# CESNET/GPUJPEG

Measured on AMD Instinct MI355X. Metric: Mpix/s encode+decode (8K RGB q75), higher is better.
Workload: dtype f32

## Files before the change

### gpujpeg_amd/csrc/gj_dec_idct.hip

```cpp
#include "gj_dec_internal.h"

__global__ __launch_bounds__(256) void k_idct(const gj_geom g, int16_t* __restrict__ coefs, const float* __restrict__ qtab,
                                              uint8_t* __restrict__ planes, const int zero)
{
    if (g.fb.sizes != nullptr) {
        coefs += (size_t)blockIdx.z * g.fb.coefs;
        planes += (size_t)blockIdx.z * g.fb.coefs;
    }
    const unsigned gb = blockIdx.x * 256u + threadIdx.x;
    if (gb >= (unsigned)g.block_count) return;
    unsigned bx, by;
    const gj_comp_geom& k = g.comp[gj_block_of(g, gb, bx, by)];
    uint32_t w[32];
    {
        uint4* p = reinterpret_cast<uint4*>(coefs + (size_t)gb * 64);
#pragma unroll
        for (int r = 0; r < 8; r++) {
            const uint4 v = p[r];
            if (zero) p[r] = make_uint4(0, 0, 0, 0);
            w[r * 4] = v.x; w[r * 4 + 1] = v.y; w[r * 4 + 2] = v.z; w[r * 4 + 3] = v.w;
        }
    }
    uint32_t px[16];
    gj_idct_pk(w, qtab + k.q_table * 64, px);
// ... 84 lines not shown
    const unsigned lb = lb0 + threadIdx.x;
    const unsigned nchunk = min(256u, nb - lb0) * 8u;
    const unsigned by = lb / (unsigned)k0.blocks_x, bx = lb - by * (unsigned)k0.blocks_x;
    uint32_t pk[3][16];
#pragma unroll
    for (int c = 0; c < 3; c++) {
        uint4* src = reinterpret_cast<uint4*>(coefs + g.comp[c].data_offset + (size_t)lb0 * 64);
        uint4 w[8];
#pragma unroll
        for (int i = 0; i < 8; i++) {
            const unsigned ch = i * 256u + threadIdx.x;
            w[i] = ch < nchunk ? src[ch] : make_uint4(0, 0, 0, 0);
        }
        if (zero) {
#pragma unroll
            for (int i = 0; i < 8; i++) {
                const unsigned ch = i * 256u + threadIdx.x;
                if (ch < nchunk) src[ch] = make_uint4(0, 0, 0, 0);
            }
        }
        if (c) __syncthreads();
#pragma unroll
        for (int i = 0; i < 8; i++) {
            const unsigned ch = i * 256u + threadIdx.x;
            *reinterpret_cast<uint4*>(s_blk + (ch >> 3) * GJ_TILE_PITCH + (ch & 7u) * 16u) = w[i];
        }
        __syncthreads();
        uint32_t wb[32];
        {
            const uint4* p = reinterpret_cast<const uint4*>(s_blk + threadIdx.x * GJ_TILE_PITCH);
#pragma unroll
            for (int r = 0; r < 8; r++) {
                const uint4 v = p[r];
                wb[r * 4] = v.x; wb[r * 4 + 1] = v.y; wb[r * 4 + 2] = v.z; wb[r * 4 + 3] = v.w;
            }
        }
        gj_idct_pk(wb, s_q[c], pk[c]);
#pragma unroll
        for (int i = 0; i < 16; i++) GJ_KEEP(pk[c][i]);
    }
    gj_store_rgb444<CS_FROM, CS_TO>(g, raw, pk, lb, nb, bx, by);
}

__device__ __forceinline__ uint4* gj_slot_row(uint8_t* slot, const int lane, const int r)
{
    return reinterpret_cast<uint4*>(slot + ((uint32_t)(r << 4) ^ (((uint32_t)lane & 7u) << 4)));
}

__device__ __forceinline__ void gj_slot_put(uint8_t* slot, const uint32_t swz , const uint32_t tok)
{
    reinterpret_cast<uint16_t*>(slot)[(tok & 63u) ^ swz] = (uint16_t)(tok & 0xFFC0u);
}

template <bool MULTI>
__device__ __forceinline__ void gj_tok_to_slot(uint8_t* slot, uint16_t* stage, const int lane, const bool fast, const uint32_t S, const uint32_t start,
                                               const uint32_t cnt, const uint32_t dc, const bool in_plane, const uint4* __restrict__ plane_block,
                                               const uint16_t* __restrict__ d_tok)
{
#pragma unroll
    for (int r = 0; r < 8; r++) *gj_slot_row(slot, lane, r) = make_uint4(0, 0, 0, 0);
    if (in_plane) {
#pragma unroll
        for (int r = 0; r < 8; r++) *gj_slot_row(slot, lane, r) = plane_block[r];
    }
    const uint32_t end = start + cnt;
    const uint32_t swz = ((uint32_t)lane & 7u) << 3;
    if (fast) {
        gj_wave_sync();
        uint32_t a = start - S;
        const uint32_t b = end - S;
        for (; a + 2 <= b; a += 2) {
            const uint32_t ta = stage[a], tb = stage[a + 1];
            gj_slot_put(slot, swz, ta);
            gj_slot_put(slot, swz, tb);
        }
        if (a < b) gj_slot_put(slot, swz, stage[a]);
    } else {
        const uint32_t prev_end = (uint32_t)__builtin_amdgcn_update_dpp(0, (int)end, 0x138, 0xF, 0xF, false);
        const unsigned long long runs0 = __ballot(lane == 0 || start != prev_end);
        uint32_t total = 0, my_at = 0;
        for (unsigned long long runs = MULTI ? runs0 : 0ull; runs;) {
            const int d = __builtin_ctzll(runs);
            runs &= runs - 1;
            const int dn = runs ? __builtin_ctzll(runs) : 64;
            const uint32_t RS = (uint32_t)__builtin_amdgcn_readlane((int)start, d), RE = (uint32_t)__builtin_amdgcn_readlane((int)end, dn - 1);
            if (lane >= d && lane < dn) my_at = total + (start - (RS & ~7u));
            total += RE > (RS & ~7u) ? (RE - (RS & ~7u) + 7u) & ~7u : 0u;
            if (RE < RS) total = GJ_TOK_STAGE + 1u;
        }
        if (MULTI && total <= GJ_TOK_STAGE) {
            gj_wave_sync();
            uint32_t at = 0;
            for (unsigned long long runs = runs0; runs;) {
                const int d = __builtin_ctzll(runs);
                runs &= runs - 1;
                const int dn = runs ? __builtin_ctzll(runs) : 64;
                const uint32_t RS = (uint32_t)__builtin_amdgcn_readlane((int)start, d) & ~7u, RE = (uint32_t)__builtin_amdgcn_readlane((int)end, dn - 1);
                for (uint32_t i = (uint32_t)lane * 8u; RS + i < RE; i += 512u)
                    *reinterpret_cast<uint4*>(stage + at + i) = *reinterpret_cast<const uint4*>(d_tok + RS + i);
                at += RE > RS ? (RE - RS + 7u) & ~7u : 0u;
            }
            gj_wave_sync();
            for (uint32_t a = 0; a < cnt; a++) gj_slot_put(slot, swz, stage[my_at + a]);
        } else {
            unsigned long long runs = runs0;
            while (runs) {
                const int d = __builtin_ctzll(runs);
                runs &= runs - 1;
                const int dn = runs ? __builtin_ctzll(runs) : 64;
                const uint32_t RS = (uint32_t)__builtin_amdgcn_readlane((int)start, d), RE = (uint32_t)__builtin_amdgcn_readlane((int)end, dn - 1);
                const bool mine = lane >= d && lane < dn;
                for (uint32_t base = RS & ~7u; base < RE; base += GJ_TOK_STAGE) {
                    gj_wave_sync();
                    for (uint32_t i = (uint32_t)lane * 8u; i < GJ_TOK_STAGE && base + i < RE; i += 512u)
                        *reinterpret_cast<uint4*>(stage + i) = *reinterpret_cast<const uint4*>(d_tok + base + i);
                    gj_wave_sync();
                    if (mine) {
                        const uint32_t b = min(end, base + GJ_TOK_STAGE);
                        for (uint32_t a = max(start, base); a < b; a++) gj_slot_put(slot, swz, stage[a - base]);
                    }
                }
            }
        }
    }
    if (!in_plane) *reinterpret_cast<uint16_t*>(slot + ((lane & 7) << 4)) = (uint16_t)dc;
    gj_wave_sync();
}

struct __attribute__((aligned(16))) GjTokLds {
    uint8_t blk[256 * 128];
    uint16_t stage[4][GJ_TOK_STAGE];
    float q[2][3][64];
};

__device__ __forceinline__ void gj_tok_tables(GjTokLds& s, const gj_geom& g, const float* __restrict__ qtab)
{
    if (threadIdx.x < 192) {
        const float q = qtab[g.comp[threadIdx.x >> 6].q_table * 64 + (threadIdx.x & 63)];
        s.q[0][threadIdx.x >> 6][threadIdx.x & 63] = (threadIdx.x & 63) ? q * 0.015625f : q;
        s.q[1][threadIdx.x >> 6][threadIdx.x & 63] = q;
    }
}

__device__ __forceinline__ void gj_tok_idct3(GjTokLds& s, const gj_geom& g, const int16_t* __restrict__ coefs, const uint16_t* __restrict__ d_tok,
                                             const unsigned lb, const uint32_t (&start)[3], const uint32_t (&cd)[3], uint32_t (&pk)[3][16])
{
    const int lane = threadIdx.x & 63;
    uint8_t* slot = s.blk + threadIdx.x * 128;
    uint16_t* stage = s.stage[threadIdx.x >> 6];
    GjTokRange cur = gj_tok_fetch(d_tok, start[0], gj_rec_count(cd[0]), lane);
#pragma unroll
    for (int c = 0; c < 3; c++) {
        const bool fast = cur.fast;
        const uint32_t S = cur.S;
        if (fast) {
            *reinterpret_cast<uint4*>(stage + lane * 8) = cur.t0;
            if (lane * 8 + 512 < GJ_TOK_STAGE) *reinterpret_cast<uint4*>(stage + lane * 8 + 512) = cur.t1;
        }
        if (c < 2) cur = gj_tok_fetch(d_tok, start[c + 1], gj_rec_count(cd[c + 1]), lane);
        const bool in_plane = (int32_t)cd[c] < 0;
        gj_tok_to_slot<false>(slot, stage, lane, fast, S, start[c], gj_rec_count(cd[c]), cd[c] & 0xFFFFu, in_plane,
                       reinterpret_cast<const uint4*>(coefs + g.comp[c].data_offset + (size_t)lb * 64), d_tok);
        uint32_t wb[32];
#pragma unroll
        for (int r = 0; r < 8; r++) {
            const uint4 v = *gj_slot_row(slot, lane, r);
            wb[r * 4] = v.x; wb[r * 4 + 1] = v.y; wb[r * 4 + 2] = v.z; wb[r * 4 + 3] = v.w;
        }
        gj_idct_pk(wb, s.q[in_plane ? 1 : 0][c], pk[c]);
#pragma unroll
        for (int i = 0; i < 16; i++) GJ_KEEP(pk[c][i]);
    }
}

template <int CS_FROM, int CS_TO>
__global__ __launch_bounds__(256, 4) void k_idct_tok_rgb444(const gj_geom g, const int16_t* __restrict__ coefs, const uint2* __restrict__ d_rec,
                                                            const uint16_t* __restrict__ d_tok, const uint32_t tok_cap,
                                                            const float* __restrict__ qtab, uint8_t* __restrict__ raw)
{
    if (g.fb.sizes != nullptr) {
        const size_t z = blockIdx.z;
        coefs += z * g.fb.coefs; d_rec += z * g.fb.rec; d_tok += z * g.fb.tok;
        raw += z * g.fb.raw;
    }
    __shared__ GjTokLds s;
    gj_tok_tables(s, g, qtab);
    const gj_comp_geom& k0 = g.comp[0];
    const unsigned nb = (unsigned)(k0.blocks_x * k0.blocks_y);
    const unsigned lb = blockIdx.x * 256u + threadIdx.x;
    const unsigned by = lb / (unsigned)k0.blocks_x, bx = lb - by * (unsigned)k0.blocks_x;
    uint32_t start[3], cd[3];
#pragma unroll
    for (int c = 0; c < 3; c++) gj_tok_record(g, d_rec, tok_cap, lb < nb, lb, c, start[c], cd[c]);
    __syncthreads();
    uint32_t pk[3][16];
    gj_tok_idct3(s, g, coefs, d_tok, lb, start, cd, pk);
    gj_store_rgb444<CS_FROM, CS_TO>(g, raw, pk, lb, nb, bx, by);
}

template <int CS_FROM, int CS_TO, bool BATCH>
__global__ __launch_bounds__(256, 4) void k_idct_tok_region_rgb444(const gj_geom g, const gj_geom gr, const gj_region rg_in, const int16_t* __restrict__ coefs,
                                                                   const uint2* __restrict__ d_rec, const uint16_t* __restrict__ d_tok,
                                                                   const uint32_t tok_cap, const float* __restrict__ qtab, uint8_t* __restrict__ raw)
{
    if (BATCH) {
        const size_t z = blockIdx.z;
        coefs += z * g.fb.coefs; d_rec += z * g.fb.rec; d_tok += z * g.fb.tok;
        raw += z * g.fb.raw;
    }
    const gj_region_frame& rg = BATCH ? rg_in.d_frames[blockIdx.z] : rg_in.frame;
    __shared__ GjTokLds s;
    gj_tok_tables(s, g, qtab);
    const int lane = threadIdx.x & 63;
    const unsigned cbx = (unsigned)(rg.bx1[0] - rg.bx0[0]), cby = (unsigned)(rg.by1[0] - rg.by0[0]);
    const unsigned pieces = (cbx + 63u) / 64u;
    const unsigned gw = blockIdx.x * 4u + (threadIdx.x >> 6);
    const unsigned crow = gw / pieces, piece = gw - crow * pieces;
    const unsigned in_piece = crow < cby ? min(64u, cbx - piece * 64u) : 0u;
    const bool valid = (unsigned)lane < in_piece;
    const unsigned fby = (unsigned)rg.by0[0] + min(crow, cby - 1u);
    const unsigned fbx = (unsigned)rg.bx0[0] + piece * 64u + (valid ? (unsigned)lane : (in_piece ? in_piece - 1u : 0u));
    const unsigned lb = fby * (unsigned)g.comp[0].blocks_x + fbx;
    uint32_t start[3], cd[3];
#pragma unroll
    for (int c = 0; c < 3; c++) gj_tok_record(g, d_rec, tok_cap, true, lb, c, start[c], cd[c]);
    if (!valid) {
#pragma unroll
        for (int c = 0; c < 3; c++) {
            start[c] += gj_rec_count(cd[c]);
            cd[c] = 0;
        }
    }
    __syncthreads();
    uint32_t pk[3][16];
    gj_tok_idct3(s, g, coefs, d_tok, lb, start, cd, pk);
    if (!valid) return;
    const int W = gr.width, H = gr.height;
    const size_t pitch = (size_t)W * 3 + gr.width_padding;
    const int x0 = (int)(fbx * 8u) - rg.x, y0 = (int)(fby * 8u) - rg.y;
    const bool inside = x0 >= 0 && x0 + 8 <= W;
#pragma unroll
    for (int r = 0; r < 8; r++) {
        uint32_t px[6] = {0, 0, 0, 0, 0, 0};
        const uint32_t c0[2] = {pk[0][2 * r], pk[0][2 * r + 1]}, c1[2] = {pk[1][2 * r], pk[1][2 * r + 1]}, c2[2] = {pk[2][2 * r], pk[2][2 * r + 1]};
        gj_store_pair<CS_FROM, CS_TO, 0>(c0, c1, c2, px);
        gj_store_pair<CS_FROM, CS_TO, 2>(c0, c1, c2, px);
        gj_store_pair<CS_FROM, CS_TO, 4>(c0, c1, c2, px);
        gj_store_pair<CS_FROM, CS_TO, 6>(c0, c1, c2, px);
        const int y = y0 + r;
        if (y >= 0 && y < H) {
            uint8_t* row = raw + (size_t)y * pitch;
            uint8_t* p = row + (ptrdiff_t)x0 * 3;
            if (inside && (reinterpret_cast<uintptr_t>(p) & 3) == 0) {
                uint32_t* q = reinterpret_cast<uint32_t*>(p);
#pragma unroll
                for (int i = 0; i < 6; i++) q[i] = px[i];
            } else {
#pragma unroll
                for (int byte = 0; byte < 24; byte++) {
                    const int x = x0 + byte / 3;
                    if (x >= 0 && x < W) row[(size_t)x * 3 + byte % 3] = (uint8_t)(px[byte >> 2] >> ((byte & 3) * 8));
                }
            }
        }
        __builtin_amdgcn_sched_barrier(0);
    }
}

__global__ __launch_bounds__(256, 4) void k_idct_tok_uyvy422(const gj_geom g, const int16_t* __restrict__ coefs, const uint2* __restrict__ d_rec,
                                                             const uint16_t* __restrict__ d_tok, const uint32_t tok_cap,
                                                             const float* __restrict__ qtab, uint8_t* __restrict__ raw)
{
    if (g.fb.sizes != nullptr) {
        const size_t z = blockIdx.z;
        coefs += z * g.fb.coefs; d_rec += z * g.fb.rec; d_tok += z * g.fb.tok;
        raw += z * g.fb.raw;
    }
    __shared__ GjTokLds s;
    gj_tok_tables(s, g, qtab);
    const gj_comp_geom& kc = g.comp[1];
    const unsigned nm = (unsigned)(kc.blocks_x * kc.blocks_y);
    const int p = threadIdx.x & 3;
    const unsigned m = blockIdx.x * 64u + (threadIdx.x >> 2);
    const unsigned my = m / (unsigned)kc.blocks_x, mx = m - my * (unsigned)kc.blocks_x;
    const int c = p < 2 ? 0 : p - 1;
    const int lane = threadIdx.x & 63;
    uint8_t* slot = s.blk + threadIdx.x * 128;
    uint16_t* stage = s.stage[threadIdx.x >> 6];
    uint32_t start = 0, cnt = 0, dc = 0;
    bool in_plane = false;
    if (m < nm) {
        const uint2 r = d_rec[(size_t)m * 4 + p];
        const uint32_t cd = gj_rec_pack(r, tok_cap);
        start = r.x;
        cnt = gj_rec_count(cd);
        dc = cd & 0xFFFFu;
        in_plane = (int32_t)cd < 0;
    }
    const GjTokRange tr = gj_tok_fetch(d_tok, start, cnt, lane);
    if (tr.fast) {
        *reinterpret_cast<uint4*>(stage + lane * 8) = tr.t0;
        if (lane * 8 + 512 < GJ_TOK_STAGE) *reinterpret_cast<uint4*>(stage + lane * 8 + 512) = tr.t1;
    }
    __syncthreads();
    const size_t blk = p < 2 ? (size_t)my * g.comp[0].blocks_x + 2 * mx + p : (size_t)m;
    gj_tok_to_slot<true>(slot, stage, lane, tr.fast, tr.S, start, cnt, dc, in_plane,
                   reinterpret_cast<const uint4*>(coefs + g.comp[c].data_offset + (m < nm ? blk : 0) * 64), d_tok);
    uint32_t wb[32];
#pragma unroll
    for (int r = 0; r < 8; r++) {
        const uint4 v = *gj_slot_row(slot, lane, r);
        wb[r * 4] = v.x; wb[r * 4 + 1] = v.y; wb[r * 4 + 2] = v.z; wb[r * 4 + 3] = v.w;
    }
    uint32_t px[16];
    gj_idct_pk(wb, s.q[in_plane ? 1 : 0][c], px);

    const size_t pitch = (size_t)g.width * 2 + g.width_padding;
    const bool interior = m < nm && (mx * 16 + 16 <= (unsigned)g.width) && (my * 8 + 8 <= (unsigned)g.height);
    const bool aligned = ((pitch | (size_t)raw) & 7) == 0;
    const uint32_t sel_uv = (p & 1) ? 0x07030602u : 0x05010400u;
#pragma unroll
    for (int r = 0; r < 8; r++) {
        const int a0 = (int)px[2 * r], a1 = (int)px[2 * r + 1];
        const uint32_t y00 = (uint32_t)__builtin_amdgcn_update_dpp(0, a0, 0x00, 0xF, 0xF, false), y01 = (uint32_t)__builtin_amdgcn_update_dpp(0, a1, 0x00, 0xF, 0xF, false);
// ... 167 lines not shown
bool gj_is_uyvy422(const gj_geom& g)
{
    return g.pixel_format == GJ_PF_422_P1020 && g.comp_count == 3 &&
           (g.color_space == g.color_space_internal || g.color_space == GJ_CS_NONE || g.color_space_internal == GJ_CS_NONE) &&
           g.comp[0].samp_h == 2 && g.comp[0].samp_v == 1 && g.comp[1].samp_h == 1 && g.comp[1].samp_v == 1 && g.comp[2].samp_h == 1 &&
           g.comp[2].samp_v == 1 && g.comp[0].blocks_x == 2 * g.comp[1].blocks_x && g.comp[0].blocks_y == g.comp[1].blocks_y &&
           g.comp[2].blocks_x == g.comp[1].blocks_x && g.comp[2].blocks_y == g.comp[1].blocks_y;
}

gj_idct_tok_t gj_idct_tok_for(const gj_geom& g)
{
    if (!g.interleaved) return gj_idct_tok_kernel(g);
    if (gj_is_uyvy422(g) && g.blocks_per_mcu == 4 && g.mcu_count == g.comp[1].blocks_x * g.comp[1].blocks_y && g.mcu_comp[0] == 0 && g.mcu_comp[1] == 0 &&
        g.mcu_comp[2] == 1 && g.mcu_comp[3] == 2 && g.mcu_bx[0] == 0 && g.mcu_bx[1] == 1)
        return k_idct_tok_uyvy422;
    return nullptr;
}

extern "C" int gj_hip_decode_uses_planes(const gj_geom* g, int use_fused)
{
    return !(use_fused && (gj_is_uyvy422(*g) || gj_idct_fused_kernel(*g) != nullptr));
}

static void gj_launch_postprocess(const gj_geom& g, const gj_dec_job* job, hipStream_t st, const unsigned frames)
{
    if (g.no_transform) {
        hipLaunchKernelGGL(k_copy_planes_out, dim3(2048, 1, frames), dim3(256), 0, st, g, job->d_planes, job->d_raw);
    } else {
        const unsigned n = (unsigned)g.raw_width * (unsigned)g.height;
        hipLaunchKernelGGL(k_postprocess, dim3((n + 255) / 256, 1, frames), dim3(256), 0, st, g, job->d_planes, job->d_raw);
    }
}

void gj_launch_idct(const gj_dec_job* job, hipStream_t st, gj_idct_tok_t idct_tok, gj_event_t* ev)
{
    const gj_geom& g = job->g;
    const bool tokens = idct_tok != nullptr;
    const unsigned frames = job->batch.count > 1 ? job->batch.count : 1u;
    int path = 0;
    const char* what = "idct / postprocess";
    if (job->region.on) {
        gj_launch_idct_region(job, st, tokens, ev);
        path = tokens ? 4 : 3;
        what = job->region.d_frames ? "idct / postprocess (batch of regions)" : "idct / postprocess (region)";
    } else if (job->scale > 1) {
        const bool done = gj_launch_idct_scaled(job, st, tokens);
        if (ev) GJ_HIP_CHECK(hipEventRecord((hipEvent_t)ev[2], st));
        if (!done) gj_launch_postprocess(job->gs, job, st, frames);
        path = done ? 2 : 1;
        what = "idct / postprocess (reduced size)";
    } else if (tokens) {
        const unsigned nb = g.interleaved ? (unsigned)g.block_count : (unsigned)(g.comp[0].blocks_x * g.comp[0].blocks_y);
        hipLaunchKernelGGL(idct_tok, dim3((nb + 255) / 256, 1, frames), dim3(256), 0, st, g, job->d_coefs, (const uint2*)job->d_blkrec, (const uint16_t*)job->d_tok, job->tok_cap,
                           job->d_qtabf, job->d_raw);
        if (ev) GJ_HIP_CHECK(hipEventRecord((hipEvent_t)ev[2], st));
    } else if (job->use_fused && gj_is_uyvy422(g)) {
        const unsigned nm = (unsigned)(g.comp[1].blocks_x * g.comp[1].blocks_y);
        hipLaunchKernelGGL(k_idct_fused_uyvy422, dim3((nm + 255) / 256, 1, frames), dim3(256), 0, st, g, job->d_coefs, job->d_qtabf, job->d_raw, job->zero_coefs);
        if (ev) GJ_HIP_CHECK(hipEventRecord((hipEvent_t)ev[2], st));
    } else if (gj_idct_fused_t fused = job->use_fused ? gj_idct_fused_kernel(g) : nullptr) {
        const unsigned nb = (unsigned)(g.comp[0].blocks_x * g.comp[0].blocks_y);
        hipLaunchKernelGGL(fused, dim3((nb + 255) / 256, 1, frames), dim3(256), 0, st, g, job->d_coefs, job->d_qtabf, job->d_raw, job->zero_coefs);
        if (ev) GJ_HIP_CHECK(hipEventRecord((hipEvent_t)ev[2], st));
    } else {
        hipLaunchKernelGGL(k_idct, dim3(((unsigned)g.block_count + 255) / 256, 1, frames), dim3(256), 0, st, g, job->d_coefs, job->d_qtabf,
                           job->d_planes, job->zero_coefs);
        if (job->flipped) hipLaunchKernelGGL(k_flip_planes, dim3(1024), dim3(256), 0, st, g, job->d_planes);
        if (ev) GJ_HIP_CHECK(hipEventRecord((hipEvent_t)ev[2], st));
        gj_launch_postprocess(g, job, st, frames);
    }
    gj_debug_stage(job->tune.debug_sync != 0, st, what);
    if (job->channel_remap) {
        const gj_geom& go = job->scale > 1 || job->region.on ? job->gs : g;
        const unsigned n = (unsigned)go.width * (unsigned)go.height;
        hipLaunchKernelGGL(k_channel_remap, dim3((n + 255) / 256), dim3(256), 0, st, go, job->d_raw, job->channel_remap & 0xFFFFu);
    }
    if (job->idct_path) *job->idct_path = path;
}
```

### gpujpeg_amd/csrc/gj_dec_internal.h

```cpp
#pragma once
#include <hip/hip_runtime.h>
#include <stdio.h>
#include <stdlib.h>

#include "gj_device.h"
#include "gj_hip.h"

static inline void gj_debug_stage(const bool on, hipStream_t st, const char* what)
{
    if (!on) return;
    const hipError_t e = hipStreamSynchronize(st);
    fprintf(stderr, "[GPUJPEG] [Debug] %s: %s\n", what, hipGetErrorString(e));
}

void gj_launch_marker_table_deferred(const gj_dec_job* job, hipStream_t st);
bool gj_tok_folds_table(const gj_dec_job* job);
bool gj_par_folds_table(const gj_dec_job* job);

void gj_launch_huffman_serial(const gj_dec_job* job, hipStream_t st);
void gj_launch_huffman_par(const gj_dec_job* job, hipStream_t st);
void gj_launch_huffman_seq(const gj_dec_job* job, hipStream_t st, bool tokens);
void gj_launch_huffman_tok(const gj_dec_job* job, hipStream_t st);

struct GjBatchPlan {
// ... 141 lines not shown
        if (regular && tid < S) {
            uint32_t st = (uint32_t)F.begin;
            if (tid > 0) {
                const uint32_t* const fp = f_o + (tid - 1) * 6;
                st = fp[0] + 2u + (((fp[3] & 0xFFu) << 8) | ((fp[3] >> 8) & 0xFFu));
            }
            hs->scan_start[tid] = st;
            hs->scan_end[tid] = f_o[tid * 6];
        }
    }
    if (tid == 0) {
        F.h_maxlen[blockIdx.x] = give_up ? 0u : *f_max;
        if (give_up) F.hsum->rst_irregular = 1u;
    }
    __syncthreads();
    return !give_up;
}

static inline bool gj_is_rgb444(const gj_geom& g)
{
    if (g.pixel_format != GJ_PF_444_P012 || g.comp_count != 3) return false;
    for (int c = 0; c < 3; c++)
        if (g.comp[c].samp_h != 1 || g.comp[c].samp_v != 1) return false;
    return true;
}
#define GJ_COLOR_PAIRS(X) \
    X(GJ_CS_NONE, GJ_CS_NONE) X(GJ_CS_BT601_256, GJ_CS_RGB) X(GJ_CS_BT601, GJ_CS_RGB) X(GJ_CS_BT709, GJ_CS_RGB) X(GJ_CS_RGB, GJ_CS_BT601_256)
static inline int gj_color_pair(const gj_geom& g)
{
    const int from = g.color_space_internal, to = g.color_space;
    if (from == to || from == GJ_CS_NONE || to == GJ_CS_NONE) return 0;
    int i = 0;
#define GJ_X(F, T) \
    if (from == F && to == T) return i; \
    i++;
    GJ_COLOR_PAIRS(GJ_X)
#undef GJ_X
    return -1;
}

__device__ __forceinline__ int gj_block_of(const gj_geom& g, const unsigned gb, unsigned& bx, unsigned& by)
{
    int c = 0;
#pragma unroll
    for (int i = 1; i < GJ_MAX_COMP; i++)
        if (i < g.comp_count && (uint64_t)gb * 64 >= g.comp[i].data_offset) c = i;
    const gj_comp_geom& k = g.comp[c];
    const unsigned lb = gb - (unsigned)(k.data_offset / 64);
    by = lb / (unsigned)k.blocks_x;
    bx = lb - by * (unsigned)k.blocks_x;
    return c;
}

typedef void (*gj_idct_tok_t)(const gj_geom, const int16_t*, const uint2*, const uint16_t*, uint32_t, const float*, uint8_t*);
gj_idct_tok_t gj_idct_tok_for(const gj_geom& g);
bool gj_is_uyvy422(const gj_geom& g);
void gj_launch_idct(const gj_dec_job* job, hipStream_t st, gj_idct_tok_t idct_tok, gj_event_t* ev);
bool gj_idct_tok_scaled_for(const gj_geom& g);
bool gj_launch_idct_scaled(const gj_dec_job* job, hipStream_t st, bool tokens);

__device__ __forceinline__ void gj_store_pixel(const gj_geom& g, uint8_t* __restrict__ raw, const unsigned W, const unsigned H, const unsigned x,
                                               const unsigned y, const unsigned pos, int (&v)[4])
{
    if (g.comp_count == 1) {
        if (g.color_space_internal == GJ_CS_RGB) v[1] = v[2] = v[0];
        else v[1] = v[2] = 128;
    }
    gj_color_transform(g.color_space_internal, g.color_space, v[0], v[1], v[2]);
    switch (g.pixel_format) {
    case GJ_PF_U8: raw[(size_t)pos + (size_t)g.width_padding * y] = (uint8_t)v[0]; break;
    case GJ_PF_444_P012: {
        uint8_t* p = raw + (size_t)pos * 3 + (size_t)g.width_padding * y;
        p[0] = (uint8_t)v[0]; p[1] = (uint8_t)v[1]; p[2] = (uint8_t)v[2];
        break; }
    case GJ_PF_4444_P0123: {
        uint8_t* p = raw + (size_t)pos * 4 + (size_t)g.width_padding * y;
        p[0] = (uint8_t)v[0]; p[1] = (uint8_t)v[1]; p[2] = (uint8_t)v[2]; p[3] = (uint8_t)v[3];
        break; }
    case GJ_PF_444_P0P1P2:
        raw[pos] = (uint8_t)v[0]; raw[(size_t)W * H + pos] = (uint8_t)v[1]; raw[(size_t)2 * W * H + pos] = (uint8_t)v[2];
        break;
    case GJ_PF_422_P0P1P2:
        raw[pos] = (uint8_t)v[0];
        if ((x & 1) == 0) {
            raw[(size_t)W * H + pos / 2] = (uint8_t)v[1];
            raw[(size_t)W * H + (size_t)H * ((W + 1) / 2) + pos / 2] = (uint8_t)v[2];
        }
        break;
    case GJ_PF_422_P1020: {
        const size_t off = (size_t)pos * 2 + (size_t)g.width_padding * y;
        raw[off + 1] = (uint8_t)v[0];
        raw[off] = (uint8_t)((x & 1) == 0 ? v[1] : v[2]);
        break; }
    case GJ_PF_420_P0P1P2:
        raw[pos] = (uint8_t)v[0];
        if ((pos & 1) == 0 && (y & 1) == 0) {
            raw[(size_t)W * H + (size_t)(y / 2) * ((W + 1) / 2) + x / 2] = (uint8_t)v[1];
            raw[(size_t)W * H + (size_t)((H + 1) / 2 + y / 2) * ((W + 1) / 2) + x / 2] = (uint8_t)v[2];
        }
        break;
    default: break;
    }
}

void gj_launch_segment_select(const gj_dec_job* job, hipStream_t st);
void gj_launch_segment_select_batch(const gj_dec_job* job, hipStream_t st);
void gj_launch_idct_region(const gj_dec_job* job, hipStream_t st, bool tokens, gj_event_t* ev);
// ... 49 lines not shown
```

### gpujpeg_amd/csrc/gj_device.h

```cpp
#pragma once
extern "C" int gj_hip_note(int hip_error);
extern "C" void gj_hip_note_reset(void);
extern "C" int gj_hip_noted(void);
#define GJ_HIP_CHECK(call) ((void)gj_hip_note((int)(call)))
#include <hip/hip_runtime.h>
#include <stdint.h>

#include "gj_hip.h"

#define GJ_WAVE 64

#include <gj_device_asm.h>

__device__ static constexpr uint8_t GJ_ZZ[64] = {
    0,  1,  8,  16, 9,  2,  3,  10, 17, 24, 32, 25, 18, 11, 4,  5,  12, 19, 26, 33, 40, 48,
    41, 34, 27, 20, 13, 6,  7,  14, 21, 28, 35, 42, 49, 56, 57, 50, 43, 36, 29, 22, 15, 23,
    30, 37, 44, 51, 58, 59, 52, 45, 38, 31, 39, 46, 53, 60, 61, 54, 47, 55, 62, 63};

struct GjSeg {
    int comp;
    int index_in_scan;
    int mcu_first;
    int nblocks;
    int last_in_scan;
// ... 354 lines not shown
    const T d3 = c3 + c4;
    const T e4 = gj_fma<T>((T)-2.0f, c4, d3);
    const T d2 = c2 + e5;
    const T f5 = gj_fma<T>((T)-2.0f, e5, d2);
    const T e1 = d6 + c1;
    const T e6 = gj_fma<T>((T)-2.0f, d6, e1);
    const T e0 = c0 + c7;
    const T e7 = gj_fma<T>((T)-2.0f, c7, e0);
    v0 = e0; v1 = e1; v2 = d2; v3 = d3; v4 = e4; v5 = f5; v6 = e6; v7 = e7;
}

__device__ __forceinline__ void gj_idct_pk(const uint32_t (&w)[32], const float* __restrict__ qf, uint32_t (&px)[16])
{
    const gj_f2* q2 = reinterpret_cast<const gj_f2*>(qf);
    gj_f2 D[8][4];
#pragma unroll
    for (int r = 0; r < 8; r++)
#pragma unroll
        for (int cp = 0; cp < 4; cp++) {
            const uint32_t v = w[r * 4 + cp];
            D[r][cp] = gj_f2{(float)(int)(int16_t)(v & 0xFFFF), (float)((int)v >> 16)} * q2[r * 4 + cp];
        }
#pragma unroll
    for (int c = 0; c < 4; c++) {
        gj_f2 x0 = D[0][c], x1 = D[4][c], x2 = D[6][c], x3 = D[2][c], x4 = D[7][c], x5 = D[5][c], x6 = D[3][c], x7 = D[1][c];
        gj_idct8<gj_f2>(x0, x1, x2, x3, x4, x5, x6, x7);
        D[0][c] = x0; D[1][c] = x1; D[2][c] = x2; D[3][c] = x3; D[4][c] = x4; D[5][c] = x5; D[6][c] = x6; D[7][c] = x7;
        __builtin_amdgcn_sched_barrier(0);
    }
#pragma unroll
    for (int rp = 0; rp < 4; rp++) {
        gj_f2 E[8];
#pragma unroll
        for (int cp = 0; cp < 4; cp++) {
            E[2 * cp] = gj_f2{D[2 * rp][cp].x, D[2 * rp + 1][cp].x};
            E[2 * cp + 1] = gj_f2{D[2 * rp][cp].y, D[2 * rp + 1][cp].y};
        }
        gj_f2 X[8] = {E[0], E[4], E[6], E[2], E[7], E[5], E[3], E[1]};
        gj_idct8<gj_f2>(X[0], X[1], X[2], X[3], X[4], X[5], X[6], X[7]);
        uint32_t a0 = 0, a1 = 0, b0 = 0, b1 = 0;
#pragma unroll
        for (int k = 0; k < 4; k++) {
            const gj_f2 lo = X[k] + (gj_f2)128.0f, hi = X[k + 4] + (gj_f2)128.0f;
            a0 = __builtin_amdgcn_cvt_pk_u8_f32(lo.x, k, a0);
            a1 = __builtin_amdgcn_cvt_pk_u8_f32(hi.x, k, a1);
            b0 = __builtin_amdgcn_cvt_pk_u8_f32(lo.y, k, b0);
            b1 = __builtin_amdgcn_cvt_pk_u8_f32(hi.y, k, b1);
        }
        px[4 * rp] = a0; px[4 * rp + 1] = a1; px[4 * rp + 2] = b0; px[4 * rp + 3] = b1;
        __builtin_amdgcn_sched_barrier(0);
    }
}

static __global__ __launch_bounds__(256) void k_flip_planes(const gj_geom g, uint8_t* __restrict__ planes)
{
    for (int c = 0; c < g.comp_count; c++) {
        const gj_comp_geom& k = g.comp[c];
        const unsigned wd = (unsigned)k.data_width / 4, half = (unsigned)k.data_height / 2;
        uint32_t* p = reinterpret_cast<uint32_t*>(planes + k.data_offset);
        for (unsigned i = blockIdx.x * 256u + threadIdx.x; i < wd * half; i += gridDim.x * 256u) {
            const unsigned y = i / wd, x = i - y * wd;
            uint32_t* a = p + (size_t)y * wd + x;
            uint32_t* b = p + (size_t)((unsigned)k.data_height - 1 - y) * wd + x;
            const uint32_t t = *a;
            *a = *b;
            *b = t;
        }
    }
}

static __global__ __launch_bounds__(256) void k_channel_remap(const gj_geom g, uint8_t* __restrict__ raw, const uint32_t map)
{
    const unsigned W = (unsigned)g.width, H = (unsigned)g.height;
    const unsigned pos = blockIdx.x * 256u + threadIdx.x;
    if (pos >= W * H) return;
    const unsigned y = pos / W;
    uint8_t* ch[4] = {nullptr, nullptr, nullptr, nullptr};
    switch (g.pixel_format) {
    case GJ_PF_U8: ch[0] = raw + (size_t)pos + (size_t)g.width_padding * y; break;
    case GJ_PF_444_P012:
        for (int c = 0; c < 3; c++) ch[c] = raw + (size_t)pos * 3 + (size_t)g.width_padding * y + c;
        break;
    case GJ_PF_4444_P0123:
        for (int c = 0; c < 4; c++) ch[c] = raw + (size_t)pos * 4 + (size_t)g.width_padding * y + c;
        break;
    default:
        for (int c = 0; c < 3; c++) ch[c] = raw + (size_t)c * W * H + pos;
        break;
    }
    const uint8_t fill = g.pixel_format == GJ_PF_U8 ? 128 : 0;
    uint8_t in[8] = {ch[0] ? *ch[0] : (uint8_t)0, ch[1] ? *ch[1] : fill, ch[2] ? *ch[2] : fill, ch[3] ? *ch[3] : (uint8_t)0, 0xFF, 0, 0, 0};
#pragma unroll
    for (int c = 0; c < 4; c++)
        if (ch[c]) *ch[c] = in[(map >> (4 * c)) & 7];
}
```

### gpujpeg_amd/csrc/gj_runtime.hip

```cpp
#include <hip/hip_runtime.h>
#include <stdlib.h>
#include <string.h>

#include <cstdio>
#include <cstring>
#include <mutex>

#include "gj_hip.h"

static thread_local hipError_t g_last = hipSuccess;

static int chk(hipError_t e)
{
    if (e != hipSuccess) {
        g_last = e;
        return -1;
    }
    return 0;
}

extern "C" {

int gj_hip_note(int hip_error) { return chk((hipError_t)hip_error); }
void gj_hip_note_reset(void) { g_last = hipSuccess; }
// ... 117 lines not shown
    if (chk(hipStreamSynchronize((hipStream_t)st))) return -1;
    if (chk(hipMemcpyAsync(d, s, n, hipMemcpyDeviceToHost, lane)) || chk(hipEventRecord((hipEvent_t)done, lane))) return -1;
    return chk(hipEventSynchronize((hipEvent_t)done));
}
gj_stream_t gj_hip_lane_begin(int download, size_t bytes_each, gj_stream_t st)
{
    hipStream_t lane = gj_lane(download ? 1 : 0, bytes_each);
    if (!lane) return st;
    if (download && chk(hipStreamSynchronize((hipStream_t)st))) return st;
    return (gj_stream_t)lane;
}
int gj_hip_lane_end(gj_stream_t lane, gj_stream_t st, gj_event_t done)
{
    if (lane == st) return 0;
    if (chk(hipEventRecord((hipEvent_t)done, (hipStream_t)lane))) return -1;
    return chk(hipEventSynchronize((hipEvent_t)done));
}
int gj_hip_memset(void* d, int v, size_t n, gj_stream_t st) { return chk(hipMemsetAsync(d, v, n, (hipStream_t)st)); }
int gj_hip_stream_sync(gj_stream_t st) { return chk(hipStreamSynchronize((hipStream_t)st)); }

int gj_hip_is_device_ptr(const void* p)
{
    hipPointerAttribute_t a;
    std::memset(&a, 0, sizeof a);
    if (hipPointerGetAttributes(&a, p) != hipSuccess) {
        (void)hipGetLastError();
        return 0;
    }
    return a.type == hipMemoryTypeDevice ? 1 : 0;
}

gj_event_t gj_hip_event_create(void)
{
    hipEvent_t e = nullptr;
    if (chk(hipEventCreate(&e))) return nullptr;
    return (gj_event_t)e;
}
void gj_hip_event_destroy(gj_event_t e)
{
    if (e) (void)hipEventDestroy((hipEvent_t)e);
}
int gj_hip_event_record(gj_event_t e, gj_stream_t s) { return chk(hipEventRecord((hipEvent_t)e, (hipStream_t)s)); }
float gj_hip_event_elapsed_ms(gj_event_t a, gj_event_t b)
{
    float ms = 0.0f;
    if (hipEventSynchronize((hipEvent_t)b) != hipSuccess) return 0.0f;
    if (hipEventElapsedTime(&ms, (hipEvent_t)a, (hipEvent_t)b) != hipSuccess) return 0.0f;
    return ms;
}

}

static std::mutex g_tune_mutex;
static gj_tuning g_tune = { 0,  -1,  -1, 0, 0, 0, 0,  -1, 0, 0, 0, 0, 0, 0, 0, 0, 0, 0, 0, 0};
static const char* const g_tune_names[] = {"GPUJPEG_NO_FUSED", "GPUJPEG_HOST_SCAN", "GJ_ENC_NO_WHOLE422", "GJ_DEC_TOKENS", "GJ_DEC_NO_TOKENS", "GJ_DEC_ENTROPY", "GJ_DEC_G",
                                           "GJ_DEC_SUB", "GJ_DEC_NO_SPEC", "GJ_DEC_SEQ", "GJ_DEC_DEBUG_SYNC", "GJ_DEC_TOK_NOCOOP", "GJ_SCAN_SHAPE", "GJ_ENC_BLOCKS",
                                           "GJ_HOST_TIMING", "GJ_DEC_BALANCE", "GJ_ENC_SPLIT", "GJ_ENC_TAIL", "GJ_DEC_FILL", "GJ_ENC_OUT_CAP", "GJ_COPY_LANES", nullptr};
static bool gj_tune_apply(gj_tuning* t, const char* name, const char* v)
{
    const auto is = [&](const char* n) { return std::strcmp(name, n) == 0; };
    const int num = std::atoi(v);
    if (is("GPUJPEG_NO_FUSED")) t->no_fused = 1;
    else if (is("GPUJPEG_HOST_SCAN")) t->host_scan = 1;
    else if (is("GJ_ENC_NO_WHOLE422")) t->enc_no_whole422 = 1;
    else if (is("GJ_DEC_TOKENS")) { if (v[0] == '1') t->dec_tokens = 1; }
    else if (is("GJ_DEC_NO_TOKENS")) t->dec_tokens = 0;
    else if (is("GJ_DEC_ENTROPY")) t->dec_serial = v[0] == 's';
    else if (is("GJ_DEC_G")) t->dec_batch = num;
    else if (is("GJ_DEC_SUB")) t->dec_sub = num;
    else if (is("GJ_DEC_NO_SPEC")) t->dec_no_spec = 1;
    else if (is("GJ_DEC_SEQ")) t->dec_seq = v[0] == '1' ? 1 : 2;
    else if (is("GJ_DEC_DEBUG_SYNC")) t->debug_sync = v[0] == '1';
    else if (is("GJ_DEC_TOK_NOCOOP")) t->dec_tok_nocoop = v[0] == '1';
    else if (is("GJ_SCAN_SHAPE")) t->scan_shape = num;
    else if (is("GJ_ENC_BLOCKS")) t->enc_by_blocks = num;
    else if (is("GJ_HOST_TIMING")) t->host_timing = v[0] == '1';
    else if (is("GJ_DEC_BALANCE")) t->dec_balance = v[0] == '1';
    else if (is("GJ_ENC_SPLIT")) t->enc_split = num;
    else if (is("GJ_ENC_TAIL")) t->enc_tail = num;
    else if (is("GJ_DEC_FILL")) t->dec_fill = num;
    else if (is("GJ_ENC_OUT_CAP")) t->enc_out_cap = num;
    else if (is("GJ_COPY_LANES")) {
        std::lock_guard<std::mutex> lk(g_lane_mutex);
        g_lanes_enabled = !(v[0] == '0' && v[1] == 0);
        g_lane_min_bytes = num > 0 ? (size_t)num << 20 : (size_t)1 << 20;
    } else return false;
    return true;
}
extern "C" int gj_hip_tuning_setting(const char* setting)
{
    std::lock_guard<std::mutex> lk(g_tune_mutex);
    if (setting == nullptr) {
        g_tune = gj_tuning{0, -1, -1, 0, 0, 0, 0, -1, 0, 0, 0, 0, 0, 0, 0, 0, 0, 0, 0, 0};
        std::lock_guard<std::mutex> lk2(g_lane_mutex);
        g_lanes_enabled = 1;
        g_lane_min_bytes = (size_t)1 << 20;
        return 0;
    }
    char name[40];
    const char* eq = std::strchr(setting, '=');
    const size_t n = eq ? (size_t)(eq - setting) : std::strlen(setting);
    if (n == 0 || n >= sizeof name) return -1;
    std::memcpy(name, setting, n);
    name[n] = 0;
    return gj_tune_apply(&g_tune, name, eq ? eq + 1 : "") ? 0 : -1;
}
extern "C" const char* const* gj_hip_tuning_names(int* count)
{
    *count = (int)(sizeof g_tune_names / sizeof g_tune_names[0]) - 1;
    return g_tune_names;
}
extern "C" void gj_hip_tuning_defaults(gj_tuning* t)
{
    {
        std::lock_guard<std::mutex> lk(g_tune_mutex);
        *t = g_tune;
    }
#ifdef GJ_TUNING_ENV
    for (const char* n : g_tune_names)
        if (n != nullptr)
            if (const char* e = getenv(n)) gj_tune_apply(t, n, e);
#endif
}
```

### include/gj_hip.h

```cpp
#ifndef GJ_HIP_H
#define GJ_HIP_H

#include <stddef.h>
#include <stdint.h>

#ifdef __cplusplus
extern "C" {
#endif

#define GJ_HIP_API __attribute__((visibility("default")))

typedef void* gj_stream_t;
typedef void* gj_event_t;

GJ_HIP_API int gj_hip_device_count(void);
GJ_HIP_API int gj_hip_get_device(int* device);
GJ_HIP_API int gj_hip_set_device(int device);
GJ_HIP_API int gj_hip_device_reset(void);
GJ_HIP_API int gj_hip_device_props(int device, char name[256], int* major, int* minor, size_t* global_mem, size_t* shared_mem,
                        int* regs_per_block, int* cu_count);
GJ_HIP_API int gj_hip_cu_count(void);
GJ_HIP_API int gj_hip_runtime_version(int* driver, int* runtime);
GJ_HIP_API const char* gj_hip_last_error(void);

// ... 45 lines not shown
    const uint32_t* sizes;
    uint64_t jpeg, raw;
    uint64_t coefs, tok, rec;
    uint32_t seg;
    uint32_t frames;
} gj_frame_strides;

typedef struct gj_geom {
    int width, height, width_padding;
    int pixel_format, color_space, color_space_internal;
    int comp_count, interleaved, restart_interval;
    int max_h, max_v;
    int mcu_count;
    int mcu_count_x;
    int segment_count;
    int scan_count;
    int blocks_per_mcu;
    int seg_blocks;
    int block_count;
    int raw_width;
    int no_transform;
    uint64_t data_size;
    uint64_t raw_size;
    gj_comp_geom comp[GJ_MAX_COMP];
    uint8_t mcu_comp[GJ_MAX_MCU_BLOCKS];
    uint8_t mcu_bx[GJ_MAX_MCU_BLOCKS];
    uint8_t mcu_by[GJ_MAX_MCU_BLOCKS];
    uint8_t mcu_prev[GJ_MAX_MCU_BLOCKS];
    gj_frame_strides fb;
} gj_geom;

#define GJ_CODER_LUT_OFFSET 1024
#define GJ_CODER_LUT_WORDS 544
typedef struct gj_tuning {
    int no_fused;
    int enc_split;
    int enc_tail;
    int dec_balance;
    int host_timing;
    int host_scan;
    int enc_no_whole422;
    int dec_tokens;
    int dec_serial;
    int dec_batch;
    int dec_sub;
    int dec_no_spec;
    int dec_seq;
    int debug_sync;
    int scan_shape;
    int dec_tok_nocoop;
    int enc_by_blocks;
    int dec_fill;
    int enc_out_cap;
    int dec_careful;
} gj_tuning;
GJ_HIP_API void gj_hip_tuning_defaults(gj_tuning* t);
GJ_HIP_API int gj_hip_tuning_setting(const char* setting);
GJ_HIP_API const char* const* gj_hip_tuning_names(int* count);

typedef struct gj_batch {
    uint32_t count;
    uint64_t raw;
    uint64_t jpeg;
    uint64_t temp;
    uint64_t coefs;
    uint64_t tok;
    uint64_t rec;
    uint32_t seg;
    uint32_t tail;
    uint32_t scratch;
    uint32_t maxlen;
    const uint32_t* d_sizes;
} gj_batch;

typedef struct gj_enc_job {
    gj_geom g;
    const uint8_t* d_raw;
    uint8_t* d_planes;
    int16_t* d_coefs;
    const float* d_fwd_q[2];
    const uint32_t* d_huff_lut;
    uint8_t* d_temp;
    uint32_t* d_seg_bytes;
    uint32_t* d_seg_ff;
    uint32_t* d_seg_out;
    uint8_t* d_jpeg;
    uint64_t jpeg_capacity;
    uint32_t* d_result;
    uint32_t* h_result;
    uint32_t* d_tail;
    int tail_set;
    uint64_t* d_scan_partial;
    uint32_t epoch;
    gj_tuning tune;
    const uint8_t* d_scan_hdr;
    uint32_t scan_hdr_offset[GJ_MAX_COMP + 1];
    uint32_t scan_info_payload[GJ_MAX_COMP];
    uint32_t main_hdr_size;
    int segment_info;
    int use_fused;
    int keep_coefs;
    int flipped;
    uint32_t channel_remap;
    gj_batch batch;
    int stage;
    uint32_t* d_huff_freq;
// ... 136 lines not shown
```

Measured before the change: 171,200.

## Add sparse 4x4-corner IDCT path for chroma blocks in token decode kernel

Adds a wave-uniform check in the RGB444 token IDCT kernel that detects when every Cb/Cr block in the wave has nonzero coefficients only in the top-left 4x4 corner. Such waves use a reduced IDCT that reads half the slot rows and skips multiplies on zero inputs. The chroma components are now processed before luma so their token fetches can be issued up front. This adds ballot and scan overhead for every wave and a new GJ_IDCT_DENSE knob to disable the path. It also adds a sparse IDCT whose numerical equivalence to the full transform depends on the hand-derived constants being correct.

Measured after the change: 176,000 (median of 6 runs). 1.03x the previous value.

```diff
diff --git a/gpujpeg_amd/csrc/gj_dec_idct.hip b/gpujpeg_amd/csrc/gj_dec_idct.hip
--- a/gpujpeg_amd/csrc/gj_dec_idct.hip
+++ b/gpujpeg_amd/csrc/gj_dec_idct.hip
@@ -160,20 +160,25 @@
     reinterpret_cast<uint16_t*>(slot)[(tok & 63u) ^ swz] = (uint16_t)(tok & 0xFFC0u);
 }
 
-template <bool MULTI>
+template <bool MULTI, bool CORNER = false>
 __device__ __forceinline__ void gj_tok_to_slot(uint8_t* slot, uint16_t* stage, const int lane, const bool fast, const uint32_t S, const uint32_t start,
                                                const uint32_t cnt, const uint32_t dc, const bool in_plane, const uint4* __restrict__ plane_block,
                                                const uint16_t* __restrict__ d_tok)
 {
-#pragma unroll
-    for (int r = 0; r < 8; r++) *gj_slot_row(slot, lane, r) = make_uint4(0, 0, 0, 0);
-    if (in_plane) {
+    if (CORNER) {
+#pragma unroll
+        for (int r = 0; r < 4; r++) *reinterpret_cast<uint2*>(gj_slot_row(slot, lane, r)) = make_uint2(0, 0);
+    } else {
+#pragma unroll
+        for (int r = 0; r < 8; r++) *gj_slot_row(slot, lane, r) = make_uint4(0, 0, 0, 0);
+    }
+    if (!CORNER && in_plane) {
 #pragma unroll
         for (int r = 0; r < 8; r++) *gj_slot_row(slot, lane, r) = plane_block[r];
     }
     const uint32_t end = start + cnt;
     const uint32_t swz = ((uint32_t)lane & 7u) << 3;
-    if (fast) {
+    if (CORNER || fast) {
         gj_wave_sync();
         uint32_t a = start - S;
         const uint32_t b = end - S;
@@ -231,7 +236,7 @@
             }
         }
     }
-    if (!in_plane) *reinterpret_cast<uint16_t*>(slot + ((lane & 7) << 4)) = (uint16_t)dc;
+    if (CORNER || !in_plane) *reinterpret_cast<uint16_t*>(slot + ((lane & 7) << 4)) = (uint16_t)dc;
     gj_wave_sync();
 }
 
@@ -250,41 +255,121 @@
     }
 }
 
+__device__ __forceinline__ void gj_tok_stage(uint16_t* stage, const int lane, const GjTokRange& r)
+{
+    if (r.fast) {
+        *reinterpret_cast<uint4*>(stage + lane * 8) = r.t0;
+        if (lane * 8 + 512 < GJ_TOK_STAGE) *reinterpret_cast<uint4*>(stage + lane * 8 + 512) = r.t1;
+    }
+}
+
+template <bool CORNER>
+__device__ __forceinline__ void gj_tok_component(GjTokLds& s, const gj_geom& g, const int16_t* __restrict__ coefs, const uint16_t* __restrict__ d_tok,
+                                                 const unsigned lb, const int c, const bool fast, const uint32_t S, const uint32_t start, const uint32_t cd,
+                                                 uint32_t (&px)[16])
+{
+    const int lane = threadIdx.x & 63;
+    uint8_t* slot = s.blk + threadIdx.x * 128;
+    const bool in_plane = !CORNER && (int32_t)cd < 0;
+    gj_tok_to_slot<false, CORNER>(slot, s.stage[threadIdx.x >> 6], lane, fast, S, start, gj_rec_count(cd), cd & 0xFFFFu, in_plane,
+                                  reinterpret_cast<const uint4*>(coefs + g.comp[c].data_offset + (size_t)lb * 64), d_tok);
+    uint32_t wb[32];
+    if (CORNER) {
+#pragma unroll
+        for (int r = 0; r < 4; r++) {
+            const uint2 v = *reinterpret_cast<const uint2*>(gj_slot_row(slot, lane, r));
+            wb[r * 4] = v.x; wb[r * 4 + 1] = v.y;
+        }
+        gj_idct_pk_corner4(wb, s.q[0][c], px);
+    } else {
+#pragma unroll
+        for (int r = 0; r < 8; r++) {
+            const uint4 v = *gj_slot_row(slot, lane, r);
+            wb[r * 4] = v.x; wb[r * 4 + 1] = v.y; wb[r * 4 + 2] = v.z; wb[r * 4 + 3] = v.w;
+        }
+        gj_idct_pk(wb, s.q[in_plane ? 1 : 0][c], px);
+    }
+#pragma unroll
+    for (int i = 0; i < 16; i++) GJ_KEEP(px[i]);
+}
+
 __device__ __forceinline__ void gj_tok_idct3(GjTokLds& s, const gj_geom& g, const int16_t* __restrict__ coefs, const uint16_t* __restrict__ d_tok,
                                              const unsigned lb, const uint32_t (&start)[3], const uint32_t (&cd)[3], uint32_t (&pk)[3][16])
 {
     const int lane = threadIdx.x & 63;
-    uint8_t* slot = s.blk + threadIdx.x * 128;
     uint16_t* stage = s.stage[threadIdx.x >> 6];
     GjTokRange cur = gj_tok_fetch(d_tok, start[0], gj_rec_count(cd[0]), lane);
 #pragma unroll
     for (int c = 0; c < 3; c++) {
         const bool fast = cur.fast;
         const uint32_t S = cur.S;
-        if (fast) {
-            *reinterpret_cast<uint4*>(stage + lane * 8) = cur.t0;
-            if (lane * 8 + 512 < GJ_TOK_STAGE) *reinterpret_cast<uint4*>(stage + lane * 8 + 512) = cur.t1;
-        }
+        gj_tok_stage(stage, lane, cur);
         if (c < 2) cur = gj_tok_fetch(d_tok, start[c + 1], gj_rec_count(cd[c + 1]), lane);
-        const bool in_plane = (int32_t)cd[c] < 0;
-        gj_tok_to_slot<false>(slot, stage, lane, fast, S, start[c], gj_rec_count(cd[c]), cd[c] & 0xFFFFu, in_plane,
-                       reinterpret_cast<const uint4*>(coefs + g.comp[c].data_offset + (size_t)lb * 64), d_tok);
-        uint32_t wb[32];
-#pragma unroll
-        for (int r = 0; r < 8; r++) {
-            const uint4 v = *gj_slot_row(slot, lane, r);
-            wb[r * 4] = v.x; wb[r * 4 + 1] = v.y; wb[r * 4 + 2] = v.z; wb[r * 4 + 3] = v.w;
-        }
-        gj_idct_pk(wb, s.q[in_plane ? 1 : 0][c], pk[c]);
-#pragma unroll
-        for (int i = 0; i < 16; i++) GJ_KEEP(pk[c][i]);
-    }
+        gj_tok_component<false>(s, g, coefs, d_tok, lb, c, fast, S, start[c], cd[c], pk[c]);
+    }
+}
+
+#ifdef GJ_HIPEMU
+extern "C" GJ_HIP_API unsigned long long gj_emu_idct_tok_waves[2];
+unsigned long long gj_emu_idct_tok_waves[2] = {0, 0};
+#endif
+
+__device__ __forceinline__ bool gj_tok_outside_corner(const GjTokRange& r, const uint32_t first, const int lane)
+{
+    const uint32_t t[8] = {r.t0.x, r.t0.y, r.t0.z, r.t0.w, r.t1.x, r.t1.y, r.t1.z, r.t1.w};
+    bool out = false;
+#pragma unroll
+    for (int k = 0; k < 16; k++) {
+        const uint32_t at = r.S + (uint32_t)lane * 8u + (uint32_t)((k >> 3) * 512 + (k & 7));
+        out |= at >= first && at < r.E && ((t[k >> 1] >> (16 * (k & 1))) & 0x24u) != 0u;
+    }
+    return out;
+}
+
+__device__ __forceinline__ void gj_tok_idct3_body(GjTokLds& s, const gj_geom& g, const int16_t* __restrict__ coefs, const uint16_t* __restrict__ d_tok,
+                                                  const unsigned lb, const uint32_t (&start)[3], const uint32_t (&cd)[3], const bool corner,
+                                                  const GjTokRange& cb, const GjTokRange& cr, uint32_t (&pk)[3][16])
+{
+    const int lane = threadIdx.x & 63;
+    uint16_t* stage = s.stage[threadIdx.x >> 6];
+    gj_tok_stage(stage, lane, cb);
+    if (corner) gj_tok_component<true>(s, g, coefs, d_tok, lb, 1, cb.fast, cb.S, start[1], cd[1], pk[1]);
+    else gj_tok_component<false>(s, g, coefs, d_tok, lb, 1, cb.fast, cb.S, start[1], cd[1], pk[1]);
+    gj_tok_stage(stage, lane, cr);
+    const GjTokRange y = gj_tok_fetch(d_tok, start[0], gj_rec_count(cd[0]), lane);
+    if (corner) gj_tok_component<true>(s, g, coefs, d_tok, lb, 2, cr.fast, cr.S, start[2], cd[2], pk[2]);
+    else gj_tok_component<false>(s, g, coefs, d_tok, lb, 2, cr.fast, cr.S, start[2], cd[2], pk[2]);
+    gj_tok_stage(stage, lane, y);
+    gj_tok_component<false>(s, g, coefs, d_tok, lb, 0, y.fast, y.S, start[0], cd[0], pk[0]);
+}
+
+__device__ __forceinline__ bool gj_tok_corner_entry(const uint16_t* __restrict__ d_tok, const uint32_t (&start)[3], const uint32_t (&cd)[3], const int dense,
+                                                    GjTokRange& cb, GjTokRange& cr)
+{
+    const int lane = threadIdx.x & 63;
+    cb = gj_tok_fetch(d_tok, start[1], gj_rec_count(cd[1]), lane);
+    cr = gj_tok_fetch(d_tok, start[2], gj_rec_count(cd[2]), lane);
+    bool corner = !dense && cb.fast && cr.fast;
+    if (corner) {
+        const bool planes = (int32_t)(cd[1] | cd[2]) < 0;
+        const uint32_t any = cb.t0.x | cb.t0.y | cb.t0.z | cb.t0.w | cb.t1.x | cb.t1.y | cb.t1.z | cb.t1.w |
+                             cr.t0.x | cr.t0.y | cr.t0.z | cr.t0.w | cr.t1.x | cr.t1.y | cr.t1.z | cr.t1.w;
+        corner = __ballot(planes || (any & 0x00240024u) != 0u) == 0ull;
+        if (!corner && __ballot(planes) == 0ull) {
+            const uint32_t first_cb = (uint32_t)__builtin_amdgcn_readlane((int)start[1], 0), first_cr = (uint32_t)__builtin_amdgcn_readlane((int)start[2], 0);
+            corner = __ballot(gj_tok_outside_corner(cb, first_cb, lane) || gj_tok_outside_corner(cr, first_cr, lane)) == 0ull;
+        }
+    }
+#ifdef GJ_HIPEMU
+    if (lane == 0) __atomic_fetch_add(&gj_emu_idct_tok_waves[corner ? 1 : 0], 1ull, __ATOMIC_RELAXED);
+#endif
+    return corner;
 }
 
 template <int CS_FROM, int CS_TO>
 __global__ __launch_bounds__(256, 4) void k_idct_tok_rgb444(const gj_geom g, const int16_t* __restrict__ coefs, const uint2* __restrict__ d_rec,
                                                             const uint16_t* __restrict__ d_tok, const uint32_t tok_cap,
-                                                            const float* __restrict__ qtab, uint8_t* __restrict__ raw)
+                                                            const float* __restrict__ qtab, uint8_t* __restrict__ raw, const int dense)
 {
     if (g.fb.sizes != nullptr) {
         const size_t z = blockIdx.z;
@@ -301,8 +386,10 @@
 #pragma unroll
     for (int c = 0; c < 3; c++) gj_tok_record(g, d_rec, tok_cap, lb < nb, lb, c, start[c], cd[c]);
     __syncthreads();
+    GjTokRange cb, cr;
     uint32_t pk[3][16];
-    gj_tok_idct3(s, g, coefs, d_tok, lb, start, cd, pk);
+    const bool corner = gj_tok_corner_entry(d_tok, start, cd, dense, cb, cr);
+    gj_tok_idct3_body(s, g, coefs, d_tok, lb, start, cd, corner, cb, cr, pk);
     gj_store_rgb444<CS_FROM, CS_TO>(g, raw, pk, lb, nb, bx, by);
 }
 
@@ -377,7 +464,7 @@
 
 __global__ __launch_bounds__(256, 4) void k_idct_tok_uyvy422(const gj_geom g, const int16_t* __restrict__ coefs, const uint2* __restrict__ d_rec,
                                                              const uint16_t* __restrict__ d_tok, const uint32_t tok_cap,
-                                                             const float* __restrict__ qtab, uint8_t* __restrict__ raw)
+                                                             const float* __restrict__ qtab, uint8_t* __restrict__ raw, const int )
 {
     if (g.fb.sizes != nullptr) {
         const size_t z = blockIdx.z;
@@ -651,7 +738,7 @@
     } else if (tokens) {
         const unsigned nb = g.interleaved ? (unsigned)g.block_count : (unsigned)(g.comp[0].blocks_x * g.comp[0].blocks_y);
         hipLaunchKernelGGL(idct_tok, dim3((nb + 255) / 256, 1, frames), dim3(256), 0, st, g, job->d_coefs, (const uint2*)job->d_blkrec, (const uint16_t*)job->d_tok, job->tok_cap,
-                           job->d_qtabf, job->d_raw);
+                           job->d_qtabf, job->d_raw, job->tune.idct_dense);
         if (ev) GJ_HIP_CHECK(hipEventRecord((hipEvent_t)ev[2], st));
     } else if (job->use_fused && gj_is_uyvy422(g)) {
         const unsigned nm = (unsigned)(g.comp[1].blocks_x * g.comp[1].blocks_y);
diff --git a/gpujpeg_amd/csrc/gj_dec_internal.h b/gpujpeg_amd/csrc/gj_dec_internal.h
--- a/gpujpeg_amd/csrc/gj_dec_internal.h
+++ b/gpujpeg_amd/csrc/gj_dec_internal.h
@@ -217,7 +217,7 @@
     return c;
 }
 
-typedef void (*gj_idct_tok_t)(const gj_geom, const int16_t*, const uint2*, const uint16_t*, uint32_t, const float*, uint8_t*);
+typedef void (*gj_idct_tok_t)(const gj_geom, const int16_t*, const uint2*, const uint16_t*, uint32_t, const float*, uint8_t*, int );
 gj_idct_tok_t gj_idct_tok_for(const gj_geom& g);
 bool gj_is_uyvy422(const gj_geom& g);
 void gj_launch_idct(const gj_dec_job* job, hipStream_t st, gj_idct_tok_t idct_tok, gj_event_t* ev);
diff --git a/gpujpeg_amd/csrc/gj_device.h b/gpujpeg_amd/csrc/gj_device.h
--- a/gpujpeg_amd/csrc/gj_device.h
+++ b/gpujpeg_amd/csrc/gj_device.h
@@ -430,6 +430,82 @@
     }
 }
 
+template <typename T>
+__device__ __forceinline__ void gj_idct8_corner4(const T v0, const T v3, const T v6, const T v7, T (&o)[8])
+{
+    const float k0 = 0.4142135623f, k1 = 0.3535533905f, k2 = 0.4619397662f, k3 = 0.1989123673f, k4 = 0.7071067811f;
+    const T b1 = v0 * (T)k1;
+    const T b0 = gj_fma<T>(v0, (T)k4, -b1);
+    const T b3 = v3 * (T)k2;
+    const T b2 = b3 * (T)k0;
+    const T b6 = v6 * (T)k0;
+    const T b5 = b6 * (T)-0.6681786379f;
+    const T b7 = v7 * (T)0.49039264f;
+    const T b4 = b7 * (T)k3;
+    const T c1 = gj_fma<T>(v0, (T)k1, b2);
+    const T c2 = gj_fma<T>((T)-2.0f, b2, c1);
+    const T c4 = b5 + b4;
+    const T c5 = gj_fma<T>((T)2.0f, b5, -c4);
+    const T c7 = b6 + b7;
+    const T c6 = gj_fma<T>((T)-2.0f, b6, c7);
+    const T c0 = b3 + b0;
+    const T c3 = gj_fma<T>((T)-2.0f, b3, c0);
+    const T d5 = gj_fma<T>(c6, (T)k0, c5);
+    const T d6 = gj_fma<T>(d5, (T)-k4, c6);
+    const T e5 = gj_fma<T>(d6, (T)k0, d5);
+    const T d3 = c3 + c4;
+    const T e4 = gj_fma<T>((T)-2.0f, c4, d3);
+    const T d2 = c2 + e5;
+    const T f5 = gj_fma<T>((T)-2.0f, e5, d2);
+    const T e1 = d6 + c1;
+    const T e6 = gj_fma<T>((T)-2.0f, d6, e1);
+    const T e0 = c0 + c7;
+    const T e7 = gj_fma<T>((T)-2.0f, c7, e0);
+    o[0] = e0; o[1] = e1; o[2] = d2; o[3] = d3; o[4] = e4; o[5] = f5; o[6] = e6; o[7] = e7;
+}
+
+__device__ __forceinline__ void gj_idct_pk_corner4(const uint32_t (&w)[32], const float* __restrict__ qf, uint32_t (&px)[16])
+{
+    const gj_f2* q2 = reinterpret_cast<const gj_f2*>(qf);
+    gj_f2 D[8][2];
+#pragma unroll
+    for (int c = 0; c < 2; c++) {
+        gj_f2 x[4];
+#pragma unroll
+        for (int r = 0; r < 4; r++) {
+            const uint32_t v = w[r * 4 + c];
+            x[r] = gj_f2{(float)(int)(int16_t)(v & 0xFFFF), (float)((int)v >> 16)} * q2[r * 4 + c];
+        }
+        gj_f2 o[8];
+        gj_idct8_corner4<gj_f2>(x[0], x[2], x[3], x[1], o);
+#pragma unroll
+        for (int r = 0; r < 8; r++) D[r][c] = o[r];
+        __builtin_amdgcn_sched_barrier(0);
+    }
+#pragma unroll
+    for (int rp = 0; rp < 4; rp++) {
+        gj_f2 E[4];
+#pragma unroll
+        for (int cp = 0; cp < 2; cp++) {
+            E[2 * cp] = gj_f2{D[2 * rp][cp].x, D[2 * rp + 1][cp].x};
+            E[2 * cp + 1] = gj_f2{D[2 * rp][cp].y, D[2 * rp + 1][cp].y};
+        }
+        gj_f2 X[8];
+        gj_idct8_corner4<gj_f2>(E[0], E[2], E[3], E[1], X);
+        uint32_t a0 = 0, a1 = 0, b0 = 0, b1 = 0;
+#pragma unroll
+        for (int k = 0; k < 4; k++) {
+            const gj_f2 lo = X[k] + (gj_f2)128.0f, hi = X[k + 4] + (gj_f2)128.0f;
+            a0 = __builtin_amdgcn_cvt_pk_u8_f32(lo.x, k, a0);
+            a1 = __builtin_amdgcn_cvt_pk_u8_f32(hi.x, k, a1);
+            b0 = __builtin_amdgcn_cvt_pk_u8_f32(lo.y, k, b0);
+            b1 = __builtin_amdgcn_cvt_pk_u8_f32(hi.y, k, b1);
+        }
+        px[4 * rp] = a0; px[4 * rp + 1] = a1; px[4 * rp + 2] = b0; px[4 * rp + 3] = b1;
+        __builtin_amdgcn_sched_barrier(0);
+    }
+}
+
 static __global__ __launch_bounds__(256) void k_flip_planes(const gj_geom g, uint8_t* __restrict__ planes)
 {
     for (int c = 0; c < g.comp_count; c++) {
diff --git a/gpujpeg_amd/csrc/gj_runtime.hip b/gpujpeg_amd/csrc/gj_runtime.hip
--- a/gpujpeg_amd/csrc/gj_runtime.hip
+++ b/gpujpeg_amd/csrc/gj_runtime.hip
@@ -193,10 +193,10 @@
 }
 
 static std::mutex g_tune_mutex;
-static gj_tuning g_tune = { 0,  -1,  -1, 0, 0, 0, 0,  -1, 0, 0, 0, 0, 0, 0, 0, 0, 0, 0, 0, 0};
+static gj_tuning g_tune = { 0,  -1,  -1, 0, 0, 0, 0,  -1, 0, 0, 0, 0, 0, 0, 0, 0, 0, 0, 0, 0, 0};
 static const char* const g_tune_names[] = {"GPUJPEG_NO_FUSED", "GPUJPEG_HOST_SCAN", "GJ_ENC_NO_WHOLE422", "GJ_DEC_TOKENS", "GJ_DEC_NO_TOKENS", "GJ_DEC_ENTROPY", "GJ_DEC_G",
                                            "GJ_DEC_SUB", "GJ_DEC_NO_SPEC", "GJ_DEC_SEQ", "GJ_DEC_DEBUG_SYNC", "GJ_DEC_TOK_NOCOOP", "GJ_SCAN_SHAPE", "GJ_ENC_BLOCKS",
-                                           "GJ_HOST_TIMING", "GJ_DEC_BALANCE", "GJ_ENC_SPLIT", "GJ_ENC_TAIL", "GJ_DEC_FILL", "GJ_ENC_OUT_CAP", "GJ_COPY_LANES", nullptr};
+                                           "GJ_HOST_TIMING", "GJ_DEC_BALANCE", "GJ_ENC_SPLIT", "GJ_ENC_TAIL", "GJ_DEC_FILL", "GJ_ENC_OUT_CAP", "GJ_IDCT_DENSE", "GJ_COPY_LANES", nullptr};
 static bool gj_tune_apply(gj_tuning* t, const char* name, const char* v)
 {
     const auto is = [&](const char* n) { return std::strcmp(name, n) == 0; };
@@ -221,6 +221,7 @@
     else if (is("GJ_ENC_TAIL")) t->enc_tail = num;
     else if (is("GJ_DEC_FILL")) t->dec_fill = num;
     else if (is("GJ_ENC_OUT_CAP")) t->enc_out_cap = num;
+    else if (is("GJ_IDCT_DENSE")) t->idct_dense = v[0] == '1';
     else if (is("GJ_COPY_LANES")) {
         std::lock_guard<std::mutex> lk(g_lane_mutex);
         g_lanes_enabled = !(v[0] == '0' && v[1] == 0);
@@ -232,7 +233,7 @@
 {
     std::lock_guard<std::mutex> lk(g_tune_mutex);
     if (setting == nullptr) {
-        g_tune = gj_tuning{0, -1, -1, 0, 0, 0, 0, -1, 0, 0, 0, 0, 0, 0, 0, 0, 0, 0, 0, 0};
+        g_tune = gj_tuning{0, -1, -1, 0, 0, 0, 0, -1, 0, 0, 0, 0, 0, 0, 0, 0, 0, 0, 0, 0, 0};
         std::lock_guard<std::mutex> lk2(g_lane_mutex);
         g_lanes_enabled = 1;
         g_lane_min_bytes = (size_t)1 << 20;
diff --git a/include/gj_hip.h b/include/gj_hip.h
--- a/include/gj_hip.h
+++ b/include/gj_hip.h
@@ -121,6 +121,7 @@
     int enc_by_blocks;
     int dec_fill;
     int enc_out_cap;
+    int idct_dense;
     int dec_careful;
 } gj_tuning;
 GJ_HIP_API void gj_hip_tuning_defaults(gj_tuning* t);
```
